# i2nico/MDAnalysis-MPI

Hardware: AMD Instinct MI355X
Metric: atom-frames/sec (RMSF) + achieved HBM GB/s fraction (higher is better)
Workload: dtype f64

## Files before the change

### mdanalysis-mpi_amd/csrc/rmsf_kernels.hip

```cpp
#include <hip/hip_runtime.h>

#include <algorithm>
#include <cmath>
#include <cstdint>
#include <cstring>
#include <mutex>
#include <string>
#include <type_traits>
#include <unordered_map>
#include <vector>

#include "rmsf_hip.h"
#include "rmsf_device.h"

#define RMSF_EXPORT __attribute__((visibility("default")))
#ifndef RMSF_SHIFTED_SUMS
#define RMSF_SHIFTED_SUMS 1
#endif

namespace {

thread_local std::string g_err;

int fail(int code, const std::string &msg) {
  g_err = msg;
  return code;
}

int hip_fail(const char *what, hipError_t e) {
  return fail(RMSF_EHIP, std::string(what) + ": " + hipGetErrorString(e));
}

#define HIP_TRY(expr)                                  \
  do {                                                 \
    hipError_t e_ = (expr);                            \
    if (e_ != hipSuccess) return hip_fail(#expr, e_);  \
  } while (0)

int after_launch(const char *what) {
  hipError_t e = hipGetLastError();
  if (e != hipSuccess) return hip_fail(what, e);
  return RMSF_OK;
}

inline hipStream_t S(void *stream) { return reinterpret_cast<hipStream_t>(stream); }

constexpr int kBlock = 256;
constexpr int kStats = 16;
constexpr int64_t kAccumBlocks = 3584;
constexpr int64_t kAccumBlocksAtom = 4608;
constexpr int64_t kStatsGroups = 3072;
constexpr int64_t kStatsRound = 768;
constexpr int64_t kStatsRoundUnits = 768 * 160;
constexpr int64_t kStatsMinUnits = 1;

constexpr int kCoefN = RMSF_MAX_SPLIT_FRAMES;
struct WCoef {
// ... 978 lines not shown
      if (MODE == RMSF_MODE_WELFORD) {
        const int64_t cs = PLANES ? ps : 1;
        float x = p[0], y = p[cs], z = p[2 * cs];
        if (ALIGN) apply_xform(x, y, z, xform + f0 * kXform, rc0, rc1, rc2);
        sh[0] = (double)x, sh[1] = (double)y, sh[2] = (double)z;
      }
      accum_span<MODE, ALIGN, U, PLANES>(p + (int64_t)s0 * fstride, fstride, s1 - s0,
                                         ALIGN ? xform + (f0 + s0) * kXform : nullptr, rc0, rc1, rc2, sh, m, q, ps);
    }
    if (qd > 0) {
#pragma unroll
      for (int j = 0; j < 3; ++j) {
        red[((qd - 1) * NV + j) * kBlock + li] = m[j];
        if (MODE == RMSF_MODE_WELFORD) red[((qd - 1) * NV + 3 + j) * kBlock + li] = q[j];
      }
    }
    __syncthreads();
    if (qd == 0 && live) {
#pragma unroll
      for (int v = 1; v < Q; ++v) {
#pragma unroll
        for (int j = 0; j < 3; ++j) {
          m[j] += red[((v - 1) * NV + j) * kBlock + li];
          if (MODE == RMSF_MODE_WELFORD) q[j] += red[((v - 1) * NV + 3 + j) * kBlock + li];
        }
      }
      if (MODE == RMSF_MODE_WELFORD) {
        const double inv = g_coef.v[len - 1].b;
#pragma unroll
        for (int j = 0; j < 3; ++j) shifted_to_moments(m[j], q[j], sh[j], inv);
      }
      const int64_t o = slot * (kBlock * 3) + 3 * li;
      store3<MODE>(parts0 + o, parts1 + o, m, q);
    }
    __syncthreads();
    lo += len;
    ++slot;
  }
}

constexpr int kFoldBatch = 4;

__device__ __forceinline__ void shift_moments(double mu, double M2, double c, double nk, double *t1, double *t2) {
  const double d = mu - c;
  *t1 = nk * d;
  *t2 = __builtin_fma(nk, d * d, M2);
}

__device__ __forceinline__ int64_t slice_t1(int64_t j, int64_t t_slice) {
  const int64_t r = j / t_slice;
  return 2 * r * t_slice + (j - r * t_slice);
}

template <int PACK, bool FIN = false>
__global__ __launch_bounds__(kBlock) void k_fold_sk(const int64_t *__restrict__ hdr,
                                                    const double *__restrict__ parts0, int64_t n_coord,
                                                    double acc_n, double *__restrict__ acc0,
                                                    double *__restrict__ acc1, const void *__restrict__ shift,
                                                    const double *__restrict__ off3, double *__restrict__ t,
                                                    int64_t l_off, int64_t l_end, int64_t t_n, int64_t t_slice,
                                                    double *__restrict__ rmsf = nullptr, double n_total = 0.0) {
  const int64_t l = l_off + (int64_t)blockIdx.x * kBlock + threadIdx.x;
  SkPlan pl;
  pl.lanes = hdr[0];
  pl.C = hdr[1];
  pl.nf = hdr[2];
  pl.T = hdr[3];
  pl.G = (int)hdr[4];
  pl.P = (int)hdr[5];
  pl.cpl = (int)hdr[6];
  pl.mode = (int)hdr[7];
  pl.S = (int)hdr[8];
  pl.cw = (int)hdr[9];
  if (l >= pl.lanes || l >= l_end) return;
  const int cpl = pl.cpl;
  const int64_t j0 = l * cpl;
  const int nx = (int)(n_coord - j0 < cpl ? n_coord - j0 : cpl);
  const int64_t c = l / pl.cw;
  const int64_t slot_d = (int64_t)pl.cw * pl.cpl;
  const int64_t off = j0 - c * slot_d;
  const int64_t clo = c * pl.nf, chi = clo + pl.nf;
  const double *__restrict__ parts1 = parts0 + (int64_t)pl.G * pl.P * slot_d;
  const bool wel = pl.mode == RMSF_MODE_WELFORD;
  double cs[4] = {0.0, 0.0, 0.0, 0.0};
  if (PACK) {
#pragma unroll
    for (int x = 0; x < 4; ++x) {
      if (x < nx) {
        const int64_t j = j0 + x;
        double c = PACK == 1 ? (double)static_cast<const float *>(shift)[j] : static_cast<const double *>(shift)[j];
        if (off3) c += off3[j % 3];
        cs[x] = c;
      }
    }
  }
  double n1 = acc_n, mu[4] = {0.0, 0.0, 0.0, 0.0}, M[4] = {0.0, 0.0, 0.0, 0.0};
  if (acc_n > 0) {
#pragma unroll
    for (int x = 0; x < 4; ++x) {
      if (x < nx) {
        mu[x] = acc0[j0 + x];
        if (wel) M[x] = acc1[j0 + x];
      }
    }
  }
  int64_t b = clo * pl.G / pl.T;
  while (b > 0 && sk_lo(pl, b) > clo) --b;
  while (sk_lo(pl, b + 1) <= clo) ++b;
  int64_t lo = sk_lo(pl, b), hi = sk_lo(pl, b + 1), slot = b * pl.P;
  while (lo < clo) {
    int64_t cc, f0;
    lo += sk_seg_len(pl, lo, hi, &cc, &f0);
    ++slot;
  }
  for (;;) {
    int64_t sl[kFoldBatch];
    double ln[kFoldBatch];
    int n = 0;
    while (n < kFoldBatch) {
      if (lo >= hi) {
        if (++b >= pl.G) break;
        lo = sk_lo(pl, b);
        hi = sk_lo(pl, b + 1);
        slot = b * pl.P;
      }
      if (lo >= chi) break;
      int64_t cc, f0;
      const int64_t len = sk_seg_len(pl, lo, hi, &cc, &f0);
      sl[n] = slot;
      ln[n] = (double)len;
      ++n;
      lo += len;
      ++slot;
    }
    double pm[kFoldBatch][4], pq[kFoldBatch][4];
#pragma unroll
    for (int k = 0; k < kFoldBatch; ++k) {
#pragma unroll
      for (int x = 0; x < 4; ++x) {
        if (k < n && x < nx) {
          const int64_t o = sl[k] * slot_d + off + x;
          pm[k][x] = parts0[o];
          pq[k][x] = wel ? parts1[o] : 0.0;
        }
      }
    }
#pragma unroll
    for (int k = 0; k < kFoldBatch; ++k) {
      if (k < n) {
#pragma unroll
        for (int x = 0; x < 4; ++x) {
          if (x >= nx) continue;
          if (!wel) {
            mu[x] += pm[k][x];
          } else if (n1 <= 0) {
            mu[x] = pm[k][x];
            M[x] = pq[k][x];
          } else {
            const double n2 = ln[k], mu2 = pm[k][x], M2 = pq[k][x];
            const double T = n1 + n2;
            const double d = mu2 - mu[x];
            const double mun = (n1 * mu[x] + n2 * mu2) / T;
            M[x] = M[x] + M2 + (n1 * n2 / T) * (d * d);
            mu[x] = mun;
          }
        }
        if (wel) n1 = n1 <= 0 ? ln[k] : n1 + ln[k];
      }
    }
    if (n < kFoldBatch) break;
  }
#pragma unroll
  for (int x = 0; x < 4; ++x) {
    if (x < nx) {
      acc0[j0 + x] = mu[x];
      if (wel) acc1[j0 + x] = M[x];
    }
  }
  if (FIN && cpl == 3 && nx == 3) rmsf[l] = sqrt((M[0] + M[1] + M[2]) / n_total);
  if (PACK) {
    const double nk = acc_n + (double)pl.nf;
    if (t_slice > 0) {
#pragma unroll
      for (int x = 0; x < 4; ++x) {
        if (x < nx) {
          double *t1 = t + slice_t1(j0 + x, t_slice);
          shift_moments(mu[x], M[x], cs[x], nk, t1, t1 + t_slice);
        }
      }
    } else {
      double *t1 = t + (j0 - l_off * cpl), *t2 = t1 + t_n;
#pragma unroll
      for (int x = 0; x < 4; ++x)
        if (x < nx) shift_moments(mu[x], M[x], cs[x], nk, t1 + x, t2 + x);
    }
  }
// ... 186 lines not shown
        acc[12] = fma(z, r0, acc[12]);
        acc[13] = fma(z, r1, acc[13]);
        acc[14] = fma(z, r2, acc[14]);
        acc[15] = fma(x, x, fma(y, y, fma(z, z, acc[15])));
      }
    };

    const f32x4 *my = reinterpret_cast<const f32x4 *>(tile + lane * kPitch + (PLANES && VEC4 ? 0 : w * 3 * kAPW));
    auto step = [&](int64_t t0) {
      __syncthreads();
      lstore();
      __syncthreads();
      gload(t0 + kTA);
      if constexpr (DENSE != 0) dense_whole(t0);
      const int64_t ab = t0 + w * kAPW;
#pragma unroll 1
      for (int gi = 0; gi < kAPW / 4; ++gi) group(my, gi, ab + 4 * gi, 4);
    };
    gload(a_beg);
    int64_t t0 = a_beg;
    for (; t0 + kTA < a_end; t0 += kTA) step(t0);
    {
      __syncthreads();
      lstore();
      __syncthreads();
      if constexpr (DENSE != 0) dense_last(t0);
      const int64_t ab = t0 + w * kAPW;
#pragma unroll 1
      for (int gi = 0; gi < kAPW / 4; ++gi) {
        const int64_t a4 = ab + 4 * gi;
        if (a4 >= a_end) break;
        group(my, gi, a4, (int)min((int64_t)4, a_end - a4));
      }
    }
    __syncthreads();
    double *red = reinterpret_cast<double *>(tile);
#pragma unroll
    for (int j = 0; j < kStats; ++j) red[(w * kStats + j) * kTF + lane] = acc[j];
    __syncthreads();
    double *out = part + slot * (kStats * kTF);
#pragma unroll
    for (int k = 0; k < kStats * kTF / kBlock; ++k) {
      const int o = threadIdx.x + k * kBlock;
      double t = red[o];
#pragma unroll
      for (int v = 1; v < kBlock / 64; ++v) t += red[v * kStats * kTF + o];
      nt_store(t, out + o);
    }
    lo += t_hi - t_lo;
    ++slot;
  }
}

template <bool GATHER, bool MASSES, bool PLANES = false>
__global__ __launch_bounds__(kBlock) void k_qcp_frames(
    const double *__restrict__ part, StatsPlan pl, int64_t n_frames, const float *__restrict__ xyz,
    int64_t fstride, const int32_t *__restrict__ sel, const double *__restrict__ refinfo,
    double *__restrict__ xform, int64_t ps = 0) {
  const int64_t f = (int64_t)blockIdx.x * (kBlock / 64) + (threadIdx.x >> 6);
  const int lane = threadIdx.x & 63;
  if (f >= n_frames) return;
  const int64_t g = f / kTF, fl = f - g * kTF;
  const int64_t ulo = g * pl.ntiles, uhi = ulo + pl.ntiles;
  int64_t b0 = ulo * pl.G / pl.T;
  while (b0 > 0 && st_lo(pl, b0) > ulo) --b0;
  while (st_lo(pl, b0 + 1) <= ulo) ++b0;
  double s[kStats];
#pragma unroll
  for (int j = 0; j < kStats; ++j) s[j] = 0.0;
  for (int64_t b = b0 + lane; b < pl.G; b += 64) {
    const int64_t blo = st_lo(pl, b);
    if (blo >= uhi) break;
    if (st_lo(pl, b + 1) <= blo) continue;
    const int64_t seg = g - blo / pl.ntiles;
    const double *pp = part + ((int64_t)b * pl.P + seg) * (kStats * kTF) + fl;
#pragma unroll
    for (int j = 0; j < kStats; ++j) s[j] += pp[j * kTF];
  }
  wave_sum(s);
  if (lane != 0) return;

  const double nsel = refinfo[7 + 1];
  const double mtot = refinfo[7];
  const int64_t o0 = GATHER ? (PLANES ? 1 : 3) * (int64_t)sel[0] : 0;
  const int64_t cs = PLANES ? ps : 1;
  const float *fr = xyz + f * fstride;
  const double px = fr[o0], py = fr[o0 + cs], pz = fr[o0 + 2 * cs];
  const double cx = (MASSES ? s[3] : s[0]) / mtot;
  const double cy = (MASSES ? s[4] : s[1]) / mtot;
  const double cz = (MASSES ? s[5] : s[2]) / mtot;
  const double sr0 = refinfo[3], sr1 = refinfo[4], sr2 = refinfo[5];
  double A[9];
  A[0] = s[6] - cx * sr0;
  A[1] = s[7] - cx * sr1;
  A[2] = s[8] - cx * sr2;
  A[3] = s[9] - cy * sr0;
  A[4] = s[10] - cy * sr1;
  A[5] = s[11] - cy * sr2;
  A[6] = s[12] - cz * sr0;
  A[7] = s[13] - cz * sr1;
  A[8] = s[14] - cz * sr2;
  const double gmob = s[15] - 2.0 * (cx * s[0] + cy * s[1] + cz * s[2]) + nsel * (cx * cx + cy * cy + cz * cz);
  const double E0 = 0.5 * (gmob + refinfo[6]);
  double *t = xform + f * kXform;
  double rot[9], rmsd;
  qcp_solve(A, E0, nsel, rot, &rmsd);
#pragma unroll
  for (int j = 0; j < 9; ++j) t[j] = rot[j];
  t[9] = px + cx;
  t[10] = py + cy;
  t[11] = pz + cz;
  t[12] = rmsd;
  t[13] = t[14] = t[15] = 0.0;
}

constexpr int kRefBlocks = 256;
constexpr int kRefThreads = 256;
static_assert(RMSF_REFINFO_DOUBLES >= 16 + 2 * 4 * kRefBlocks, "refinfo scratch");

template <bool FROM_F32, bool GATHER>
__device__ __forceinline__ void ref_load(const float *__restrict__ frame, const double *__restrict__ avg,
                                         const int32_t *__restrict__ sel, int64_t a, double &x, double &y,
                                         double &z, double div = 1.0) {
  if (FROM_F32) {
    const float *p = frame + (GATHER ? 3 * (int64_t)sel[a] : 3 * a);
    x = (double)p[0];
    y = (double)p[1];
    z = (double)p[2];
  } else {
    x = avg[3 * a] / div;
    y = avg[3 * a + 1] / div;
    z = avg[3 * a + 2] / div;
  }
}

__device__ __forceinline__ void block_sum4(double (&v)[4], double *out) {
  __shared__ double red[kRefThreads / 64][4];
  wave_sum(v);
  const int w = threadIdx.x >> 6, lane = threadIdx.x & 63;
  if (lane == 0)
    for (int j = 0; j < 4; ++j) red[w][j] = v[j];
  __syncthreads();
  if (threadIdx.x < 4) {
    double t = 0.0;
    for (int i = 0; i < kRefThreads / 64; ++i) t += red[i][threadIdx.x];
    out[threadIdx.x] = t;
  }
}

__device__ __forceinline__ void fold_partials(const double *__restrict__ p, int nb, double (&t)[4]) {
  const int lane = threadIdx.x & 63;
  for (int j = 0; j < 4; ++j) t[j] = 0.0;
  for (int b = lane; b < nb; b += 64)
    for (int j = 0; j < 4; ++j) t[j] += p[4 * b + j];
  wave_sum(t);
}

template <bool FROM_F32, bool GATHER, bool MASSES>
__device__ __forceinline__ void ref_com_body(const float *__restrict__ frame, const double *__restrict__ avg,
                                             int64_t n_sel, const int32_t *__restrict__ sel,
                                             const double *__restrict__ masses, double *__restrict__ info, int blk,
                                             int nblk, double div = 1.0) {
  double v[4] = {0, 0, 0, 0};
  const int64_t stride = (int64_t)nblk * kRefThreads;
  for (int64_t a = (int64_t)blk * kRefThreads + threadIdx.x; a < n_sel; a += stride) {
    double x, y, z;
// ... 379 lines not shown

__global__ __launch_bounds__(kBlock) void k_synth(float *__restrict__ out, int64_t fstride, int64_t n_atoms,
                                                  int64_t f0, int64_t nf, uint64_t seed,
                                                  const double *__restrict__ motion) {
#pragma clang fp contract(off)
  const int64_t t = (int64_t)blockIdx.x * kBlock + threadIdx.x;
  if (t >= nf * n_atoms) return;
  const int64_t fl = t / n_atoms, a = t - fl * n_atoms;
  const int64_t f = f0 + fl;
  const double two24 = 5.9604644775390625e-08;
  const double two53 = 1.1102230246251565e-16;
  const double sqrt6 = 2.449489742783178;
  const double sigma = 0.2 + (double)(skey(seed, 2, (uint64_t)a, 0) >> 11) * two53 * 1.8;
  double p[3];
  for (int c = 0; c < 3; ++c) {
    const double base = (double)(skey(seed, 1, (uint64_t)a, (uint64_t)c) >> 11) * two53 * 100.0;
    const uint64_t h = skey(seed, 3, (uint64_t)f, (uint64_t)(3 * a + c));
    const uint64_t u = (h >> 40) + ((h >> 16) & 0xFFFFFFull);
    const double g = ((double)u * two24 - 1.0) * sqrt6;
    const double s = sigma * g;
    p[c] = base + s;
  }
  float *o = out + fl * fstride + 3 * a;
  if (motion) {
    const double *M = motion + 12 * f;
    const double d0 = p[0] - 50.0, d1 = p[1] - 50.0, d2 = p[2] - 50.0;
    for (int b = 0; b < 3; ++b) {
      const double e0 = d0 * M[b];
      const double e1 = d1 * M[3 + b];
      const double e2 = d2 * M[6 + b];
      const double y = ((e0 + e1) + e2) + M[9 + b];
      o[b] = (float)y;
    }
  } else {
    o[0] = (float)p[0];
    o[1] = (float)p[1];
    o[2] = (float)p[2];
  }
}

inline unsigned grid1(int64_t n) { return (unsigned)((n + kBlock - 1) / kBlock); }

StatsPlan stats_plan(int64_t n_sel, int64_t n_frames) {
  StatsPlan p;
  p.ntiles = (n_sel + kTA - 1) / kTA;
  p.ngroups = std::max<int64_t>(1, (n_frames + kTF - 1) / kTF);
  p.T = p.ntiles * p.ngroups;
  const int64_t rounds = std::min<int64_t>(kStatsGroups / kStatsRound,
                                           std::max<int64_t>(1, (p.T + kStatsRoundUnits / 2) / kStatsRoundUnits));
  p.G = (int)std::max<int64_t>(1, std::min<int64_t>(kStatsRound * rounds, p.T / kStatsMinUnits));
  const int64_t len = (p.T + p.G - 1) / p.G;
  p.P = (int)((len + p.ntiles - 1) / p.ntiles + 1);
  return p;
}

}

extern "C" {

RMSF_EXPORT int rmsf_abi_version(void) { return RMSF_ABI_VERSION; }

RMSF_EXPORT int rmsf_internal_set_error(int code, const char *msg) { return fail(code, msg ? msg : ""); }

RMSF_EXPORT const char *rmsf_last_error(void) { return g_err.c_str(); }

RMSF_EXPORT int rmsf_device_count(int *n) {
  if (!n) return fail(RMSF_EINVAL, "rmsf_device_count: null");
  HIP_TRY(hipGetDeviceCount(n));
  return RMSF_OK;
}

RMSF_EXPORT int rmsf_set_device(int dev) {
  HIP_TRY(hipSetDevice(dev));
  return RMSF_OK;
}

RMSF_EXPORT int rmsf_malloc(void **p, size_t bytes) {
  if (!p) return fail(RMSF_EINVAL, "rmsf_malloc: null");
  hipError_t e = hipMalloc(p, bytes);
  if (e != hipSuccess) return fail(RMSF_ENOMEM, std::string("hipMalloc: ") + hipGetErrorString(e));
  return RMSF_OK;
}

RMSF_EXPORT int rmsf_free(void *p) {
  HIP_TRY(hipFree(p));
  return RMSF_OK;
}

RMSF_EXPORT int rmsf_memcpy_h2d(void *d, const void *h, size_t bytes, void *stream) {
  HIP_TRY(hipMemcpyAsync(d, h, bytes, hipMemcpyHostToDevice, S(stream)));
  return RMSF_OK;
}

RMSF_EXPORT int rmsf_memcpy_d2h(void *h, const void *d, size_t bytes, void *stream) {
  HIP_TRY(hipMemcpyAsync(h, d, bytes, hipMemcpyDeviceToHost, S(stream)));
  HIP_TRY(hipStreamSynchronize(S(stream)));
  return RMSF_OK;
}

RMSF_EXPORT int rmsf_memcpy2d_d2d(void *d_dst, size_t dpitch, const void *d_src, size_t spitch, size_t width,
                                 size_t height, void *stream) {
  if (!d_dst || !d_src || width > dpitch || width > spitch) return fail(RMSF_EINVAL, "rmsf_memcpy2d_d2d: bad arguments");
  if (width == 0 || height == 0) return RMSF_OK;
  HIP_TRY(hipMemcpy2DAsync(d_dst, dpitch, d_src, spitch, width, height, hipMemcpyDeviceToDevice, S(stream)));
  return RMSF_OK;
}
// ... 97 lines not shown
  if (n_sel < 1 || n_frames < 0) return 0;
  const StatsPlan p = stats_plan(n_sel, n_frames);
  return (size_t)p.G * (size_t)p.P * kStats * kTF * sizeof(double);
}

}

namespace {

int superpose_impl(const char *who, const float *d_xyz, int64_t fstride, int64_t ps, int64_t n_frames, int64_t n_sel,
                   const int32_t *d_sel, const double *d_masses, const double *d_ref, const double *d_refinfo,
                   double *d_xform, void *d_work, size_t work_bytes, hipStream_t s, float *d_dense = nullptr,
                   int64_t dense_pitch = 0) {
  if (n_frames == 0) return RMSF_OK;
  const bool planes = ps > 0;
  if (!d_xyz || !d_ref || !d_refinfo || !d_xform || !d_work || n_sel < 1 || n_frames < 0 ||
      (planes ? (ps < (d_sel ? 1 : n_sel) || fstride < 3 * ps) : fstride < (d_sel ? 3 : 3 * n_sel)))
    return fail(RMSF_EINVAL, std::string(who) + ": bad arguments");
  const StatsPlan plan = stats_plan(n_sel, n_frames);
  if (work_bytes < rmsf_superpose_workspace_bytes(n_sel, n_frames))
    return fail(RMSF_ENOMEM, std::string(who) + ": workspace too small");
  double *part = static_cast<double *>(d_work);
  const bool g = d_sel != nullptr, m = d_masses != nullptr;
  const bool vec4 = !g && fstride % 4 == 0 && (!planes || ps % 4 == 0) &&
                    reinterpret_cast<uintptr_t>(d_xyz) % 16 == 0;
  dim3 grid((unsigned)plan.G);
  auto stats = [&](auto P) {
    constexpr bool PL = decltype(P)::value;
#define ST_LAUNCH(G, M, V) \
  hipLaunchKernelGGL((k_frame_stats<G, M, V, 1, PL>), grid, dim3(kBlock), 0, s, d_xyz, fstride, n_frames, n_sel, d_sel, d_masses, d_ref, plan, part, ps)
#define ST_DENSE(M, D) \
  hipLaunchKernelGGL((k_frame_stats<true, M, false, 3, false, D>), grid, dim3(kBlock), 0, s, d_xyz, fstride, n_frames, n_sel, d_sel, d_masses, d_ref, plan, part, ps, d_dense, dense_pitch)
    if (d_dense) {
      if constexpr (!PL) {
        const bool dv = dense_pitch % 4 == 0 && reinterpret_cast<uintptr_t>(d_dense) % 16 == 0;
        if (m && dv) ST_DENSE(true, 2);
        else if (m) ST_DENSE(true, 1);
        else if (dv) ST_DENSE(false, 2);
        else ST_DENSE(false, 1);
      }
    } else if (g && m) ST_LAUNCH(true, true, false);
    else if (g) ST_LAUNCH(true, false, false);
    else if (m && vec4) ST_LAUNCH(false, true, true);
    else if (m) ST_LAUNCH(false, true, false);
    else if (vec4) ST_LAUNCH(false, false, true);
    else ST_LAUNCH(false, false, false);
#undef ST_LAUNCH
#undef ST_DENSE
  };
  if (planes) stats(std::true_type{});
  else stats(std::false_type{});
  int rc = after_launch("k_frame_stats");
  if (rc) return rc;
  const unsigned gq = (unsigned)((n_frames + 3) / 4);
  auto qcp = [&](auto P) {
    constexpr bool PL = decltype(P)::value;
#define QCP_LAUNCH(G, M) \
  hipLaunchKernelGGL((k_qcp_frames<G, M, PL>), dim3(gq), dim3(kBlock), 0, s, part, plan, n_frames, d_xyz, fstride, d_sel, d_refinfo, d_xform, ps)
    if (g && m) QCP_LAUNCH(true, true);
    else if (g) QCP_LAUNCH(true, false);
    else if (m) QCP_LAUNCH(false, true);
    else QCP_LAUNCH(false, false);
#undef QCP_LAUNCH
  };
  if (planes) qcp(std::true_type{});
  else qcp(std::false_type{});
  return after_launch("k_qcp_frames");
}

}

extern "C" {

RMSF_EXPORT int rmsf_superpose(const float *d_xyz, int64_t fstride, int64_t n_frames, int64_t n_sel,
                               const int32_t *d_sel, const double *d_masses, const double *d_ref,
                               const double *d_refinfo, double *d_xform, void *d_work, size_t work_bytes,
                               void *stream) {
  return superpose_impl("rmsf_superpose", d_xyz, fstride, 0, n_frames, n_sel, d_sel, d_masses, d_ref, d_refinfo,
                        d_xform, d_work, work_bytes, S(stream));
}

RMSF_EXPORT int rmsf_superpose_compact(const float *d_xyz, int64_t fstride, int64_t n_frames, int64_t n_sel,
                                       const int32_t *d_sel, const double *d_masses, const double *d_ref,
                                       const double *d_refinfo, double *d_xform, void *d_work, size_t work_bytes,
                                       float *d_dense_out, int64_t dense_stride, void *stream) {
  if (!d_sel || !d_dense_out) return fail(RMSF_EINVAL, "rmsf_superpose_compact: needs a selection and an output");
  if (dense_stride == 0) dense_stride = 3 * n_sel;
  if (dense_stride < 3 * n_sel) return fail(RMSF_EINVAL, "rmsf_superpose_compact: dense_stride < 3 n_sel");
  return superpose_impl("rmsf_superpose_compact", d_xyz, fstride, 0, n_frames, n_sel, d_sel, d_masses, d_ref,
                        d_refinfo, d_xform, d_work, work_bytes, S(stream), d_dense_out, dense_stride);
}

RMSF_EXPORT int rmsf_superpose_planes(const float *d_xyz, int64_t fstride, int64_t pstride, int64_t n_frames,
                                      int64_t n_sel, const int32_t *d_sel, const double *d_masses,
                                      const double *d_ref, const double *d_refinfo, double *d_xform, void *d_work,
                                      size_t work_bytes, void *stream) {
  if (pstride < 1) return fail(RMSF_EINVAL, "rmsf_superpose_planes: plane stride < 1");
  return superpose_impl("rmsf_superpose_planes", d_xyz, fstride, pstride, n_frames, n_sel, d_sel, d_masses, d_ref,
                        d_refinfo, d_xform, d_work, work_bytes, S(stream));
}

RMSF_EXPORT int64_t rmsf_split_count(int64_t n_frames, int n_splits, int s) {
  if (n_splits < 1 || s < 0 || s >= n_splits) return -1;
  return (n_frames * (s + 1)) / n_splits - (n_frames * s) / n_splits;
}

RMSF_EXPORT int rmsf_accumulate_splits(int64_t n_sel, int64_t n_frames, int aligned) {
  if (n_frames <= 0) return 1;
  const int64_t lanes = aligned ? n_sel : (3 * n_sel + 3) / 4;
  const int64_t blocks_x = std::max<int64_t>(1, (lanes + kBlock - 1) / kBlock);
  const int64_t target = aligned ? kAccumBlocksAtom : kAccumBlocks;
// ... 64 lines not shown
  return n;
}

constexpr int kSkPerCuFlat = 2, kSkPerCuAtoms = 2, kSkPerCuAligned = 32;
constexpr int kQWel = 2, kSkPerCuSplitWel = 8, kQSum = 4, kSkPerCuSplitSum = 4;
constexpr int kSeqU = 8;
constexpr int kSeqAtomsU = 4;
constexpr int64_t kSeqAtomsMinSel = 49152;


SkPlan sk_plan(int64_t lanes, int cpl, int64_t nf, int n_groups, int mode, int per_cu, int cw = kBlock) {
  SkPlan p{};
  p.lanes = lanes;
  p.cw = cw;
  p.C = (lanes + cw - 1) / cw;
  p.nf = nf;
  p.T = p.C * nf;
  p.cpl = cpl;
  p.mode = mode;
  p.c0 = 0;
  int64_t G = n_groups > 0 ? n_groups : (int64_t)per_cu * cu_count();
  int64_t S = 0;
  if (n_groups <= 0 && p.C > G) {
    S = std::max<int64_t>((nf + kCoefN - 1) / kCoefN, (kAccumBlocks + p.C - 1) / p.C);
    S = std::min<int64_t>(S, std::max<int64_t>(1, nf / kSkMinSeg));
    G = p.C * S;
  } else if (n_groups <= 0) {
    G = std::min<int64_t>(G, std::max<int64_t>(1, p.T / kSkMinSeg));
    G = std::min<int64_t>(G, std::max<int64_t>(1, p.C * kSkMaxSegsPerChunk));
  }
  G = std::max<int64_t>(1, std::min<int64_t>({G, p.T, (int64_t)INT32_MAX}));
  p.G = (int)G;
  const int64_t W = (p.T + G - 1) / G;
  p.P = (int)((W + kCoefN - 1) / kCoefN + (W - 1) / nf + 2);
  if (S > 0 && G == p.C * S) {
    p.S = (int)S;
    if (nf % S == 0) p.P = (int)((nf / S + kCoefN - 1) / kCoefN);
  }
  p.Cs = p.C;
  return p;
}

size_t sk_bytes(const SkPlan &p, bool two) {
  const size_t part = (size_t)p.G * (size_t)p.P * (size_t)p.cw * (size_t)p.cpl * sizeof(double);
  return kSkHdr * sizeof(int64_t) + part * (two ? 2 : 1);
}

bool flat_layout(const float *d_xyz, int64_t fstride, int64_t n_sel, const int32_t *d_sel, const double *d_xform,
                 int mode) {
  return !d_xform && !d_sel && mode == RMSF_MODE_WELFORD && (3 * n_sel) % 4 == 0 && fstride % 4 == 0 &&
         reinterpret_cast<uintptr_t>(d_xyz) % 16 == 0;
}

int fold_shift_launch(const int64_t *hdr, const double *p0, int64_t n_coord, int64_t acc_n, double *acc0, double *acc1,
                      const void *shift, int shift_is_f32, const double *off3, double *t, int64_t l0, int64_t l1,
                      int64_t t_n, int64_t threads, hipStream_t s, int64_t t_slice = 0) {
  if (shift_is_f32)
    hipLaunchKernelGGL(k_fold_sk<1>, dim3(grid1(threads)), dim3(kBlock), 0, s, hdr, p0, n_coord, (double)acc_n, acc0,
                       acc1, shift, off3, t, l0, l1, t_n, t_slice);
  else
    hipLaunchKernelGGL(k_fold_sk<2>, dim3(grid1(threads)), dim3(kBlock), 0, s, hdr, p0, n_coord, (double)acc_n, acc0,
                       acc1, shift, off3, t, l0, l1, t_n, t_slice);
  return after_launch("k_fold_sk");
}

double merge_weight(int64_t n1, int64_t n2) {
  const int64_t T = n1 + n2;
  return T > 0 ? (double)(n1 * n2) / (double)T : 0.0;
}

std::vector<std::pair<int, int>> reduce_schedule(int n_parts, int order) {
  std::vector<std::pair<int, int>> st;
  if (order == RMSF_MERGE_RANK) {
    for (int i = 1; i < n_parts; ++i) st.push_back({0, i});
    return st;
  }
  for (int64_t mask = 1; mask < n_parts; mask <<= 1)
    for (int64_t r = 0; r + mask < n_parts; r += 2 * mask) st.push_back({(int)r, (int)(r + mask)});
  return st;
}

}

extern "C" {

RMSF_EXPORT size_t rmsf_accumulate_balanced_workspace_bytes(int64_t n_sel, int64_t n_frames, int n_groups) {
  if (n_sel < 1 || n_frames < 1) return 0;
  size_t m = 0;
  for (int per_cu : {kSkPerCuFlat, kSkPerCuAtoms, kSkPerCuAligned, kSkPerCuSplitWel, kSkPerCuSplitSum}) {
    m = std::max(m, sk_bytes(sk_plan((3 * n_sel + 3) / 4, 4, n_frames, n_groups, RMSF_MODE_WELFORD, per_cu), true));
    m = std::max(m, sk_bytes(sk_plan(n_sel, 3, n_frames, n_groups, RMSF_MODE_WELFORD, per_cu), true));
  }
  return m;
}

RMSF_EXPORT int rmsf_accumulate_balanced(const float *d_xyz, int64_t fstride, int64_t n_frames, int64_t n_sel,
                                         const int32_t *d_sel, const double *d_xform, const double *d_refinfo,
                                         int mode, int n_groups, void *d_work, size_t work_bytes, void *stream) {
  if (mode != RMSF_MODE_WELFORD && mode != RMSF_MODE_SUM)
    return fail(RMSF_EINVAL, "rmsf_accumulate_balanced: bad mode");
  if (!d_xyz || !d_work || n_sel < 1 || n_frames < 1 || fstride < (d_sel ? 3 : 3 * n_sel) ||
      reinterpret_cast<uintptr_t>(d_work) % 16 != 0)
    return fail(RMSF_EINVAL, "rmsf_accumulate_balanced: bad arguments");
  if (d_xform && !d_refinfo) return fail(RMSF_EINVAL, "rmsf_accumulate_balanced: aligned mode needs d_refinfo");
  hipStream_t s = S(stream);
  const bool two = mode == RMSF_MODE_WELFORD;
  int64_t *hdr = static_cast<int64_t *>(d_work);
  if (flat_layout(d_xyz, fstride, n_sel, d_sel, d_xform, mode)) {
    const SkPlan pl = sk_plan(3 * n_sel / 4, 4, n_frames, n_groups, mode, kSkPerCuFlat);
    if (work_bytes < sk_bytes(pl, two)) return fail(RMSF_ENOMEM, "rmsf_accumulate_balanced: workspace too small");
    double *p0 = reinterpret_cast<double *>(hdr + kSkHdr);
    double *p1 = p0 + (size_t)pl.G * pl.P * kBlock * 4;
    hipLaunchKernelGGL((k_welford_flat_sk<4>), dim3(pl.G), dim3(kBlock), 0, s, d_xyz, fstride / 4, pl, hdr, p0, p1);
    return after_launch("k_welford_flat_sk");
  }
// ... 37 lines not shown
}

RMSF_EXPORT int rmsf_accumulate_balanced_planes(const float *d_xyz, int64_t fstride, int64_t pstride,
                                                int64_t n_frames, int64_t n_sel, const int32_t *d_sel,
                                                const double *d_xform, const double *d_refinfo, int mode,
                                                int n_groups, void *d_work, size_t work_bytes, void *stream) {
#if RMSF_SHIFTED_SUMS
  if (mode != RMSF_MODE_WELFORD && mode != RMSF_MODE_SUM)
    return fail(RMSF_EINVAL, "rmsf_accumulate_balanced_planes: bad mode");
  if (!d_xyz || !d_work || (d_xform && !d_refinfo) || n_sel < 1 || n_frames < 1 || pstride < (d_sel ? 1 : n_sel) ||
      fstride < 3 * pstride || reinterpret_cast<uintptr_t>(d_work) % 16 != 0)
    return fail(RMSF_EINVAL, "rmsf_accumulate_balanced_planes: bad arguments");
  hipStream_t s = S(stream);
  const bool two = mode == RMSF_MODE_WELFORD, g = d_sel != nullptr;
  const int per_cu = !d_xform ? kSkPerCuAtoms : two ? kSkPerCuSplitWel : kSkPerCuSplitSum;
  const SkPlan pl = sk_plan(n_sel, 3, n_frames, n_groups, mode, per_cu);
  if (work_bytes < sk_bytes(pl, two)) return fail(RMSF_ENOMEM, "rmsf_accumulate_balanced_planes: workspace too small");
  int64_t *hdr = static_cast<int64_t *>(d_work);
  double *p0 = reinterpret_cast<double *>(hdr + kSkHdr);
  double *p1 = two ? p0 + (size_t)pl.G * pl.P * kBlock * 3 : nullptr;
  if (!d_xform) {
#define SK_LAUNCH(M_, G_) \
  hipLaunchKernelGGL((k_accum_atoms_sk<M_, false, G_, 4, true>), dim3(pl.G), dim3(kBlock), 0, s, d_xyz, fstride, d_sel, nullptr, nullptr, pl, hdr, p0, p1, pstride)
    if (two && g) SK_LAUNCH(0, true);
    else if (two) SK_LAUNCH(0, false);
    else if (g) SK_LAUNCH(1, true);
    else SK_LAUNCH(1, false);
#undef SK_LAUNCH
    return after_launch("k_accum_atoms_sk");
  }
#define SPLIT_LAUNCH(M_, G_, Q_) \
  hipLaunchKernelGGL((k_accum_split_sk<M_, true, G_, 4, Q_, true>), dim3(pl.G), dim3(kBlock * Q_), 0, s, d_xyz, fstride, d_sel, d_xform, d_refinfo, pl, hdr, p0, p1, pstride)
  if (two) {
    if (g) SPLIT_LAUNCH(0, true, kQWel);
    else SPLIT_LAUNCH(0, false, kQWel);
  } else {
    if (g) SPLIT_LAUNCH(1, true, kQSum);
    else SPLIT_LAUNCH(1, false, kQSum);
  }
#undef SPLIT_LAUNCH
  return after_launch("k_accum_split_sk");
#else
  return fail(RMSF_EINVAL, "rmsf_accumulate_balanced_planes: needs the shifted-sums build");
#endif
}

RMSF_EXPORT int rmsf_fold_balanced(const void *d_work, int64_t n_coord, int mode, int64_t acc_n, double *d_acc0,
                                   double *d_acc1, void *stream) {
  if (mode != RMSF_MODE_WELFORD && mode != RMSF_MODE_SUM) return fail(RMSF_EINVAL, "rmsf_fold_balanced: bad mode");
  if (!d_work || !d_acc0 || (mode == RMSF_MODE_WELFORD && !d_acc1) || n_coord < 1 || acc_n < 0)
    return fail(RMSF_EINVAL, "rmsf_fold_balanced: bad arguments");
  const int64_t *hdr = static_cast<const int64_t *>(d_work);
  const double *p0 = reinterpret_cast<const double *>(hdr + kSkHdr);
  hipLaunchKernelGGL(k_fold_sk<0>, dim3(grid1((n_coord + 2) / 3)), dim3(kBlock), 0, S(stream), hdr, p0, n_coord,
                     (double)acc_n, d_acc0, d_acc1, nullptr, nullptr, nullptr, (int64_t)0, INT64_MAX, n_coord,
                     (int64_t)0);
  return after_launch("k_fold_sk");
}

RMSF_EXPORT int rmsf_fold_balanced_finalize(const void *d_work, int64_t n_coord, int64_t acc_n, double *d_acc0,
                                            double *d_acc1, int64_t n_total, double *d_rmsf, void *stream) {
  if (!d_work || !d_acc0 || !d_acc1 || !d_rmsf || n_coord < 3 || n_coord % 3 != 0 || acc_n < 0 || n_total < 1)
    return fail(RMSF_EINVAL, "rmsf_fold_balanced_finalize: bad arguments");
  const int64_t *hdr = static_cast<const int64_t *>(d_work);
  const double *p0 = reinterpret_cast<const double *>(hdr + kSkHdr);
  hipLaunchKernelGGL((k_fold_sk<0, true>), dim3(grid1((n_coord + 2) / 3)), dim3(kBlock), 0, S(stream), hdr, p0,
                     n_coord, (double)acc_n, d_acc0, d_acc1, nullptr, nullptr, nullptr, (int64_t)0, INT64_MAX, n_coord,
                     (int64_t)0, d_rmsf, (double)n_total);
  int rc = after_launch("k_fold_sk<FIN>");
  if (rc) return rc;
  const int64_t n_sel = n_coord / 3;
  hipLaunchKernelGGL(k_finalize_flat, dim3((unsigned)std::min<int64_t>(grid1(n_sel), 1024)), dim3(kBlock), 0,
                     S(stream), hdr, d_acc1, n_sel, (double)n_total, d_rmsf);
  return after_launch("k_finalize_flat");
}

RMSF_EXPORT int rmsf_fold_balanced_shift(const void *d_work, int64_t n_coord, int64_t acc_n, double *d_acc0,
                                         double *d_acc1, const void *d_shift, int shift_is_f32, const double *d_off3,
                                         double *d_t, void *stream) {
  if (!d_work || !d_acc0 || !d_acc1 || !d_shift || !d_t || n_coord < 1 || acc_n < 0)
    return fail(RMSF_EINVAL, "rmsf_fold_balanced_shift: bad arguments");
  const int64_t *hdr = static_cast<const int64_t *>(d_work);
  const double *p0 = reinterpret_cast<const double *>(hdr + kSkHdr);
  return fold_shift_launch(hdr, p0, n_coord, acc_n, d_acc0, d_acc1, d_shift, shift_is_f32, d_off3, d_t, 0, INT64_MAX,
                           n_coord, (n_coord + 2) / 3, S(stream));
}

RMSF_EXPORT int rmsf_fold_balanced_shift_sliced(const void *d_work, int64_t n_coord, int64_t acc_n, double *d_acc0,
                                                double *d_acc1, const void *d_shift, int shift_is_f32,
                                                const double *d_off3, int64_t slice_coords, double *d_t,
                                                void *stream) {
  if (!d_work || !d_acc0 || !d_acc1 || !d_shift || !d_t || n_coord < 1 || acc_n < 0 || slice_coords < 3 ||
      slice_coords % 3)
    return fail(RMSF_EINVAL, "rmsf_fold_balanced_shift_sliced: bad arguments");
  const int64_t *hdr = static_cast<const int64_t *>(d_work);
  const double *p0 = reinterpret_cast<const double *>(hdr + kSkHdr);
  return fold_shift_launch(hdr, p0, n_coord, acc_n, d_acc0, d_acc1, d_shift, shift_is_f32, d_off3, d_t, 0, INT64_MAX,
                           n_coord, (n_coord + 2) / 3, S(stream), slice_coords);
}

RMSF_EXPORT int rmsf_balanced_slab_chunks(const float *d_xyz, int64_t fstride, int64_t n_frames, int64_t n_sel,
                                          int64_t *h_chunks) {
  if (!h_chunks || n_sel < 1 || n_frames < 1) return fail(RMSF_EINVAL, "rmsf_balanced_slab_chunks: bad arguments");
  *h_chunks = 0;
  if (!flat_layout(d_xyz, fstride, n_sel, nullptr, nullptr, RMSF_MODE_WELFORD)) return RMSF_OK;
  const SkPlan pl = sk_plan(3 * n_sel / 4, 4, n_frames, 0, RMSF_MODE_WELFORD, kSkPerCuFlat);
  if (pl.S > 0) *h_chunks = pl.C;
  return RMSF_OK;
}

RMSF_EXPORT int rmsf_accumulate_balanced_slab(const float *d_xyz, int64_t fstride, int64_t n_frames, int64_t n_sel,
                                              int64_t c0, int64_t c1, void *d_work, size_t work_bytes,
                                              void *stream) {
  if (!d_xyz || !d_work || n_sel < 1 || n_frames < 1 || reinterpret_cast<uintptr_t>(d_work) % 16 != 0)
    return fail(RMSF_EINVAL, "rmsf_accumulate_balanced_slab: bad arguments");
  if (!flat_layout(d_xyz, fstride, n_sel, nullptr, nullptr, RMSF_MODE_WELFORD))
    return fail(RMSF_EINVAL, "rmsf_accumulate_balanced_slab: needs the flat float4 layout (no selection, aligned)");
  SkPlan pl = sk_plan(3 * n_sel / 4, 4, n_frames, 0, RMSF_MODE_WELFORD, kSkPerCuFlat);
  if (pl.S <= 0) return fail(RMSF_EINVAL, "rmsf_accumulate_balanced_slab: the plan is not chunk-aligned");
  if (c0 < 0 || c1 <= c0 || c1 > pl.C) return fail(RMSF_EINVAL, "rmsf_accumulate_balanced_slab: bad chunk range");
  if (work_bytes < sk_bytes(pl, true)) return fail(RMSF_ENOMEM, "rmsf_accumulate_balanced_slab: workspace too small");
// ... 573 lines not shown
```

Before: 545.9 billion.

## Add lane-per-frame QCP kernel and division-free segment walk in fold

The fold kernel now advances across balanced-partition blocks using an incremental quotient/remainder walk instead of recomputing sk_lo with 64-bit divisions, and it loads partials without per-element predicates by clamping indices. A new k_qcp_lanes kernel assigns one frame per lane (64 frames per wave) and has each lane reduce its partials through a bit-reversed pairwise tree. This replaces the old scheme where a whole wave reduced one frame's partials and a single lane then ran the QCP solve. Both new paths are on by default, with environment variables to select the old forms; the cost is more register use per lane and a different summation order.

```diff
diff --git a/mdanalysis-mpi_amd/csrc/rmsf_kernels.hip b/mdanalysis-mpi_amd/csrc/rmsf_kernels.hip
--- a/mdanalysis-mpi_amd/csrc/rmsf_kernels.hip
+++ b/mdanalysis-mpi_amd/csrc/rmsf_kernels.hip
@@ -3,6 +3,7 @@
 #include <algorithm>
 #include <cmath>
 #include <cstdint>
+#include <cstdlib>
 #include <cstring>
 #include <mutex>
 #include <string>
@@ -1087,7 +1088,7 @@
   return 2 * r * t_slice + (j - r * t_slice);
 }
 
-template <int PACK, bool FIN = false>
+template <int PACK, bool FIN = false, bool DIVWALK = false>
 __global__ __launch_bounds__(kBlock) void k_fold_sk(const int64_t *__restrict__ hdr,
                                                     const double *__restrict__ parts0, int64_t n_coord,
                                                     double acc_n, double *__restrict__ acc0,
@@ -1148,6 +1149,8 @@
     lo += sk_seg_len(pl, lo, hi, &cc, &f0);
     ++slot;
   }
+  const int64_t qT = pl.T / pl.G, rT = pl.T - qT * pl.G;
+  int64_t rem = pl.T * (b + 1) - hi * pl.G;
   for (;;) {
     int64_t sl[kFoldBatch];
     double ln[kFoldBatch];
@@ -1155,28 +1158,53 @@
     while (n < kFoldBatch) {
       if (lo >= hi) {
         if (++b >= pl.G) break;
-        lo = sk_lo(pl, b);
-        hi = sk_lo(pl, b + 1);
+        if constexpr (DIVWALK) {
+          lo = sk_lo(pl, b);
+          hi = sk_lo(pl, b + 1);
+        } else {
+          lo = hi;
+          hi += qT;
+          rem += rT;
+          if (rem >= pl.G) {
+            rem -= pl.G;
+            ++hi;
+          }
+        }
         slot = b * pl.P;
       }
       if (lo >= chi) break;
-      int64_t cc, f0;
-      const int64_t len = sk_seg_len(pl, lo, hi, &cc, &f0);
+      int64_t len = hi - lo;
+      if constexpr (DIVWALK) {
+        int64_t cc, f0;
+        len = sk_seg_len(pl, lo, hi, &cc, &f0);
+      } else {
+        if (chi - lo < len) len = chi - lo;
+        if (len > kCoefN) len = kCoefN;
+      }
       sl[n] = slot;
       ln[n] = (double)len;
       ++n;
       lo += len;
       ++slot;
     }
+    if (n == 0) break;
+    const double *__restrict__ second = wel ? parts1 : parts0;
     double pm[kFoldBatch][4], pq[kFoldBatch][4];
 #pragma unroll
     for (int k = 0; k < kFoldBatch; ++k) {
+      const int64_t ok = (k < n ? sl[k] : sl[0]) * slot_d + off;
 #pragma unroll
       for (int x = 0; x < 4; ++x) {
-        if (k < n && x < nx) {
-          const int64_t o = sl[k] * slot_d + off + x;
+        if constexpr (DIVWALK) {
+          if (k < n && x < nx) {
+            const int64_t o = sl[k] * slot_d + off + x;
+            pm[k][x] = parts0[o];
+            pq[k][x] = wel ? parts1[o] : 0.0;
+          }
+        } else {
+          const int64_t o = ok + (x < nx ? x : nx - 1);
           pm[k][x] = parts0[o];
-          pq[k][x] = wel ? parts1[o] : 0.0;
+          pq[k][x] = second[o];
         }
       }
     }
@@ -1469,6 +1497,27 @@
   }
 }
 
+template <bool MASSES>
+__device__ __forceinline__ void qcp_record(const double (&s)[kStats], int64_t f, double px, double py, double pz,
+                                           const double *__restrict__ refinfo, double *__restrict__ xform);
+
+template <bool GATHER, bool PLANES>
+__device__ __forceinline__ void frame_pivot(int64_t f, const float *__restrict__ xyz, int64_t fstride,
+                                            const int32_t *__restrict__ sel, int64_t ps, double &px, double &py,
+                                            double &pz) {
+  const int64_t o0 = GATHER ? (PLANES ? 1 : 3) * (int64_t)sel[0] : 0;
+  const int64_t cs = PLANES ? ps : 1;
+  const float *fr = xyz + f * fstride;
+  px = fr[o0], py = fr[o0 + cs], pz = fr[o0 + 2 * cs];
+}
+
+__device__ __forceinline__ int64_t st_first_cover(const StatsPlan &pl, int64_t ulo) {
+  int64_t b0 = ulo * pl.G / pl.T;
+  while (b0 > 0 && st_lo(pl, b0) > ulo) --b0;
+  while (st_lo(pl, b0 + 1) <= ulo) ++b0;
+  return b0;
+}
+
 template <bool GATHER, bool MASSES, bool PLANES = false>
 __global__ __launch_bounds__(kBlock) void k_qcp_frames(
     const double *__restrict__ part, StatsPlan pl, int64_t n_frames, const float *__restrict__ xyz,
@@ -1479,9 +1528,7 @@
   if (f >= n_frames) return;
   const int64_t g = f / kTF, fl = f - g * kTF;
   const int64_t ulo = g * pl.ntiles, uhi = ulo + pl.ntiles;
-  int64_t b0 = ulo * pl.G / pl.T;
-  while (b0 > 0 && st_lo(pl, b0) > ulo) --b0;
-  while (st_lo(pl, b0 + 1) <= ulo) ++b0;
+  const int64_t b0 = st_first_cover(pl, ulo);
   double s[kStats];
 #pragma unroll
   for (int j = 0; j < kStats; ++j) s[j] = 0.0;
@@ -1496,13 +1543,16 @@
   }
   wave_sum(s);
   if (lane != 0) return;
-
+  double px, py, pz;
+  frame_pivot<GATHER, PLANES>(f, xyz, fstride, sel, ps, px, py, pz);
+  qcp_record<MASSES>(s, f, px, py, pz, refinfo, xform);
+}
+
+template <bool MASSES>
+__device__ __forceinline__ void qcp_record(const double (&s)[kStats], int64_t f, double px, double py, double pz,
+                                           const double *__restrict__ refinfo, double *__restrict__ xform) {
   const double nsel = refinfo[7 + 1];
   const double mtot = refinfo[7];
-  const int64_t o0 = GATHER ? (PLANES ? 1 : 3) * (int64_t)sel[0] : 0;
-  const int64_t cs = PLANES ? ps : 1;
-  const float *fr = xyz + f * fstride;
-  const double px = fr[o0], py = fr[o0 + cs], pz = fr[o0 + 2 * cs];
   const double cx = (MASSES ? s[3] : s[0]) / mtot;
   const double cy = (MASSES ? s[4] : s[1]) / mtot;
   const double cz = (MASSES ? s[5] : s[2]) / mtot;
@@ -1529,6 +1579,80 @@
   t[11] = pz + cz;
   t[12] = rmsd;
   t[13] = t[14] = t[15] = 0.0;
+}
+
+template <bool GATHER, bool MASSES, bool PLANES = false>
+__global__ __launch_bounds__(64) void k_qcp_lanes(const double *__restrict__ part, StatsPlan pl, int64_t n_frames,
+                                                  const float *__restrict__ xyz, int64_t fstride,
+                                                  const int32_t *__restrict__ sel,
+                                                  const double *__restrict__ refinfo, double *__restrict__ xform,
+                                                  int64_t ps, int fpw) {
+  const int lane = threadIdx.x;
+  const int64_t fw = (int64_t)blockIdx.x * fpw;
+  const int64_t f = fw + lane;
+  if (lane >= fpw || f >= n_frames) return;
+  double px, py, pz;
+  frame_pivot<GATHER, PLANES>(f, xyz, fstride, sel, ps, px, py, pz);
+  const int64_t g = fw / kTF;
+  const int64_t fl = f - g * kTF;
+  const int64_t ulo = g * pl.ntiles, uhi = ulo + pl.ntiles;
+  int64_t b0 = ulo * pl.G / pl.T;
+  while (st_lo(pl, b0 + 1) <= ulo) ++b0;
+  b0 = uni64(b0);
+  const int64_t seg0 = uni64(g - st_lo(pl, b0) / pl.ntiles);
+  const int64_t bend = uni64(min((int64_t)pl.G, (uhi * pl.G + pl.T - 1) / pl.T));
+  const int nb = (int)min((int64_t)64, bend - b0);
+  int m = 0;
+  while ((1 << m) < nb) ++m;
+  const int n = 1 << m;
+  auto partial = [&](int64_t b) { return part + (b * pl.P + (b == b0 ? seg0 : 0)) * (kStats * kTF) + fl; };
+  double st[4][kStats], x[4][kStats];
+  const int nq = n >= 4 ? n / 4 : 1;
+#pragma unroll 1
+  for (int q = 0; q < nq; ++q) {
+    bool ok[4];
+#pragma unroll
+    for (int k = 0; k < 4; ++k) {
+      const int i = 4 * q + k;
+      const int L = m ? (int)(__builtin_bitreverse32((unsigned)i) >> (32 - m)) : 0;
+      ok[k] = i < n && b0 + L < bend;
+      const double *pp = partial(ok[k] ? b0 + L : b0);
+#pragma unroll
+      for (int j = 0; j < kStats; ++j) x[k][j] = pp[j * kTF];
+    }
+#pragma unroll
+    for (int k = 0; k < 4; ++k) {
+#pragma unroll
+      for (int j = 0; j < kStats; ++j) x[k][j] = ok[k] ? 0.0 + x[k][j] : 0.0;
+      if (ok[k] && n == 64) {
+        const int i = 4 * q + k;
+        const int L = (int)(__builtin_bitreverse32((unsigned)i) >> (32 - 6));
+        for (int64_t b = b0 + L + 64; b < bend; b += 64) {
+          const double *pp = partial(b);
+#pragma unroll
+          for (int j = 0; j < kStats; ++j) x[k][j] += pp[j * kTF];
+        }
+      }
+    }
+#pragma unroll
+    for (int j = 0; j < kStats; ++j) x[0][j] = (x[0][j] + x[1][j]) + (x[2][j] + x[3][j]);
+    const int c = __builtin_ctz(~(unsigned)q);
+#pragma unroll
+    for (int lev = 0; lev < 4; ++lev) {
+      if (lev < c) {
+#pragma unroll
+        for (int j = 0; j < kStats; ++j) x[0][j] = st[lev][j] + x[0][j];
+      }
+    }
+#pragma unroll
+    for (int lev = 0; lev < 4; ++lev) {
+      if (lev == c) {
+#pragma unroll
+        for (int j = 0; j < kStats; ++j) st[lev][j] = x[0][j];
+      }
+    }
+  }
+  qcp_record<MASSES>(x[0], f, px, py, pz, refinfo, xform);
 }
 
 constexpr int kRefBlocks = 256;
@@ -2014,6 +2138,14 @@
   const int64_t len = (p.T + p.G - 1) / p.G;
   p.P = (int)((len + p.ntiles - 1) / p.ntiles + 1);
   return p;
+}
+
+int qcp_frames_per_wave() {
+  if (const char *e = std::getenv("RMSF_QCP_FORM")) {
+    const int v = std::atoi(e);
+    if (v == 1 || v == 16 || v == 32 || v == 64) return v;
+  }
+  return 64;
 }
 
 }
@@ -2217,11 +2349,19 @@
   else stats(std::false_type{});
   int rc = after_launch("k_frame_stats");
   if (rc) return rc;
-  const unsigned gq = (unsigned)((n_frames + 3) / 4);
+  const int fpw = plan.G <= plan.T ? qcp_frames_per_wave() : 1;
+  const unsigned gq = fpw > 1 ? (unsigned)((n_frames + fpw - 1) / fpw) : (unsigned)((n_frames + 3) / 4);
   auto qcp = [&](auto P) {
     constexpr bool PL = decltype(P)::value;
-#define QCP_LAUNCH(G, M) \
-  hipLaunchKernelGGL((k_qcp_frames<G, M, PL>), dim3(gq), dim3(kBlock), 0, s, part, plan, n_frames, d_xyz, fstride, d_sel, d_refinfo, d_xform, ps)
+#define QCP_LAUNCH(G, M)                                                                                              \
+  do {                                                                                                                \
+    if (fpw > 1)                                                                                                      \
+      hipLaunchKernelGGL((k_qcp_lanes<G, M, PL>), dim3(gq), dim3(64), 0, s, part, plan, n_frames, d_xyz, fstride,     \
+                         d_sel, d_refinfo, d_xform, ps, fpw);                                                         \
+    else                                                                                                              \
+      hipLaunchKernelGGL((k_qcp_frames<G, M, PL>), dim3(gq), dim3(kBlock), 0, s, part, plan, n_frames, d_xyz,         \
+                         fstride, d_sel, d_refinfo, d_xform, ps);                                                     \
+  } while (0)
     if (g && m) QCP_LAUNCH(true, true);
     else if (g) QCP_LAUNCH(true, false);
     else if (m) QCP_LAUNCH(false, true);
@@ -2392,15 +2532,27 @@
          reinterpret_cast<uintptr_t>(d_xyz) % 16 == 0;
 }
 
+bool fold_divwalk() {
+  const char *e = std::getenv("RMSF_FOLD_FORM");
+  return e && std::strcmp(e, "div") == 0;
+}
+
+#define FOLD_LAUNCH(PACK, FIN, threads, s, ...)                                                          \
+  do {                                                                                                   \
+    const dim3 fg_(grid1(threads)), fb_(kBlock);                                                         \
+    if (fold_divwalk()) hipLaunchKernelGGL((k_fold_sk<PACK, FIN, true>), fg_, fb_, 0, s, __VA_ARGS__);   \
+    else hipLaunchKernelGGL((k_fold_sk<PACK, FIN, false>), fg_, fb_, 0, s, __VA_ARGS__);                 \
+  } while (0)
+
 int fold_shift_launch(const int64_t *hdr, const double *p0, int64_t n_coord, int64_t acc_n, double *acc0, double *acc1,
                       const void *shift, int shift_is_f32, const double *off3, double *t, int64_t l0, int64_t l1,
                       int64_t t_n, int64_t threads, hipStream_t s, int64_t t_slice = 0) {
   if (shift_is_f32)
-    hipLaunchKernelGGL(k_fold_sk<1>, dim3(grid1(threads)), dim3(kBlock), 0, s, hdr, p0, n_coord, (double)acc_n, acc0,
-                       acc1, shift, off3, t, l0, l1, t_n, t_slice);
+    FOLD_LAUNCH(1, false, threads, s, hdr, p0, n_coord, (double)acc_n, acc0, acc1, shift, off3, t, l0, l1, t_n,
+                t_slice, (double *)nullptr, 0.0);
   else
-    hipLaunchKernelGGL(k_fold_sk<2>, dim3(grid1(threads)), dim3(kBlock), 0, s, hdr, p0, n_coord, (double)acc_n, acc0,
-                       acc1, shift, off3, t, l0, l1, t_n, t_slice);
+    FOLD_LAUNCH(2, false, threads, s, hdr, p0, n_coord, (double)acc_n, acc0, acc1, shift, off3, t, l0, l1, t_n,
+                t_slice, (double *)nullptr, 0.0);
   return after_launch("k_fold_sk");
 }
 
@@ -2544,9 +2696,9 @@
     return fail(RMSF_EINVAL, "rmsf_fold_balanced: bad arguments");
   const int64_t *hdr = static_cast<const int64_t *>(d_work);
   const double *p0 = reinterpret_cast<const double *>(hdr + kSkHdr);
-  hipLaunchKernelGGL(k_fold_sk<0>, dim3(grid1((n_coord + 2) / 3)), dim3(kBlock), 0, S(stream), hdr, p0, n_coord,
-                     (double)acc_n, d_acc0, d_acc1, nullptr, nullptr, nullptr, (int64_t)0, INT64_MAX, n_coord,
-                     (int64_t)0);
+  FOLD_LAUNCH(0, false, (n_coord + 2) / 3, S(stream), hdr, p0, n_coord, (double)acc_n, d_acc0, d_acc1,
+              (const void *)nullptr, (const double *)nullptr, (double *)nullptr, (int64_t)0, INT64_MAX, n_coord,
+              (int64_t)0, (double *)nullptr, 0.0);
   return after_launch("k_fold_sk");
 }
 
@@ -2556,9 +2708,9 @@
     return fail(RMSF_EINVAL, "rmsf_fold_balanced_finalize: bad arguments");
   const int64_t *hdr = static_cast<const int64_t *>(d_work);
   const double *p0 = reinterpret_cast<const double *>(hdr + kSkHdr);
-  hipLaunchKernelGGL((k_fold_sk<0, true>), dim3(grid1((n_coord + 2) / 3)), dim3(kBlock), 0, S(stream), hdr, p0,
-                     n_coord, (double)acc_n, d_acc0, d_acc1, nullptr, nullptr, nullptr, (int64_t)0, INT64_MAX, n_coord,
-                     (int64_t)0, d_rmsf, (double)n_total);
+  FOLD_LAUNCH(0, true, (n_coord + 2) / 3, S(stream), hdr, p0, n_coord, (double)acc_n, d_acc0, d_acc1,
+              (const void *)nullptr, (const double *)nullptr, (double *)nullptr, (int64_t)0, INT64_MAX, n_coord,
+              (int64_t)0, d_rmsf, (double)n_total);
   int rc = after_launch("k_fold_sk<FIN>");
   if (rc) return rc;
   const int64_t n_sel = n_coord / 3;
```

Result: no change. 545.8 billion, median of 3 (-0.0%).
